# yynps737/zero-latency-yolo

Hardware: AMD Instinct MI355X
Metric: frames_per_sec (higher is better)
Workload: dtype bf16; 1 GPU; YOLOv8-nano 416x416 batch=64 throughput path (BASELINE configs[2]), bf16; engines_per_gpu=3, weights=seeded synthetic (no real weights offline), graph=True, parallelism=single GPU

## Files before the change

### zero-latency-yolo_amd/csrc/engine.cpp

```cpp
#include "zly_internal.h"
#include "weights.h"

#include <algorithm>
#include <atomic>
#include <chrono>
#include <condition_variable>
#include <deque>
#include <map>
#include <mutex>
#include <string>
#include <thread>
#include <type_traits>
#include <vector>
#include <string.h>
#include <stdio.h>
#include <stdlib.h>

namespace zly {

static thread_local std::string g_last_error;

static int fail(int code, const std::string& msg) { g_last_error = msg; return code; }

#define HIP_TRY(expr, code)                                                                        \
// ... 65 lines not shown
};

struct Plan {
    int nc = 0, N = 0;
    std::vector<Buffer> bufs;
    std::vector<Op> ops;
    std::vector<PairGroup> pairs;
    std::vector<C2fGroup> c2fs;
    DetectTail tail;
    int in_buf = -1;
    std::map<std::string, std::pair<int, int>> tap_index;
    std::map<std::string, std::pair<int, int>> tap_final;
    bool stem_fused = false;
    bool stem1 = false;
    size_t stem_w = 0, stem_b = 0, m1_w = 0, m1_b = 0, stem_w0p = 0;
    int stem_out = -1, m1_out = -1;
    int sppf_cv1 = -1, sppf_pool = -1, sppf_cv2 = -1;
    int det_stem[3] = {-1, -1, -1}, det_a[3] = {-1, -1, -1}, det_b[3] = {-1, -1, -1};
    bool det_merge_ok = false;
    int join_at = -1;
    std::vector<uint8_t> blob;
};

enum LaunchKind { LK_NONE, LK_PREPROCESS, LK_STEM, LK_STEM1, LK_CONV, LK_CONV_WSK, LK_MULTI, LK_C2F, LK_PAIR, LK_WS_PAIR, LK_SPPF_FUSED, LK_SPPF_POOL, LK_HEAD, LK_NMS };
struct Launch {
    int kind = LK_NONE;
    int covered_by = -1;
    bool hbm = true;
    ConvPlan conv{};
    WskPlan wsk{};
    C2fPlan c2f{};
    PairPlan pair{};
    WsPairPlan ws_pair{};
    int multi_ct = 0;
    int only_level = -1;
    int box_mode[3] = {0, 0, 0};
    bool pool16 = false;
    bool lb = false;
};

struct Ingest;

}

using namespace zly;

struct zly_engine : Plan {
    zly_config cfg;
    std::string weights_path;
    int dev = 0;
    int dtype = ZLY_DTYPE_BF16;
    size_t esz = 2;
    ModelFile model;

    void* d_weights = nullptr;
    float* d_head = nullptr;
    Cand* d_cand = nullptr;
    Cand* d_scratch = nullptr;
    int* d_count = nullptr;
// ... 60 lines not shown

namespace zly {

static size_t slab_bytes_of(const zly_engine* e) { return sizeof(zly_slab_header) + (size_t)e->cfg.max_dets * sizeof(zly_det); }

template <typename F> static void with_stats(zly_engine* e, F&& f) { std::lock_guard<std::mutex> lk(e->stats_mu); f(e->stats); }

static void read_switches(Switches* sw)
{
    auto on = [](const char* name) { return getenv(name) != nullptr; };
    auto num = [](const char* name, auto* out) { if (const char* v = getenv(name)) *out = (std::remove_pointer_t<decltype(out)>)atoll(v); };
    *sw = Switches();
    if (const char* cp = getenv("ZLY_CU_PART")) {
        int pi = 0, pn = 1;
        if (sscanf(cp, "%d/%d", &pi, &pn) == 2 && pn >= 1 && pn <= 8 && pi >= 0 && pi < pn) { sw->cu_part_i = pi; sw->cu_part_n = pn; sw->num_cus = 256 / pn; }
    }
    sw->no_lanes = on("ZLY_NO_LANES") || on("ZLY_CU_PART");
    sw->no_c2f = on("ZLY_NO_C2F");
    sw->no_det_merge = on("ZLY_NO_DET_MERGE");
    sw->no_tail_split = on("ZLY_NO_TAIL_SPLIT");
    num("ZLY_TAIL_BOX", &sw->tail_box);
    if (const char* v = getenv("ZLY_TAIL_BOX_MIN_CONF")) sw->tail_box_min_conf = (float)atof(v);
    sw->sppf_fused = on("ZLY_SPPF_FUSED");
    sw->pool_six_pass = on("ZLY_SPPF_POOL_LDS");
    sw->no_wsk = on("ZLY_NO_WSK");
    sw->nms_general = on("ZLY_NMS_GENERAL");
    sw->no_cout_pad = on("ZLY_NO_COUT_PAD");
    sw->no_cin_pad = on("ZLY_NO_CIN_PAD");
    sw->no_stem1 = on("ZLY_NO_STEM1");
    num("ZLY_STEM1_NW", &sw->stem1_nw);
    num("ZLY_STEM1_VAR", &sw->stem1_var);
    num("ZLY_STEM1_GRID", &sw->stem1_grid);
    num("ZLY_STEM1_TW", &sw->stem1_tw);
    num("ZLY_STEM1_TH", &sw->stem1_th);
    sw->stem1_keep_tiles = on("ZLY_STEM1_TW") || on("ZLY_STEM1_TH") || on("ZLY_STEM1_BIG_TILES");
    num("ZLY_PAIR_MIN_TILES", &sw->pair_min_tiles);
    num("ZLY_PAIR_WIDTHS", &sw->pair_widths);
    auto num_nonempty = [&](const char* name, int* out) { const char* v = getenv(name); if (v && *v) *out = atoi(v); };
    num_nonempty("ZLY_STAGE_SLOTS", &sw->stage_slots);
    num_nonempty("ZLY_STAGE_MB", &sw->stage_mb);
    num_nonempty("ZLY_INFLIGHT", &sw->inflight);
    { int d = 0; num_nonempty("ZLY_D2H_STREAM", &d); sw->d2h_stream = d != 0; }
    num("ZLY_PROFILE_INNER", &sw->profile_inner);
    if (sw->profile_inner < 1) sw->profile_inner = 1;
#ifdef ZLY_DIAG
    if (const char* v = getenv("ZLY_ABLATE_SKIP")) sw->ablate = std::string(",") + v + ",";
// ... 327 lines not shown
    p->stem1 = p->stem_fused && ch[0] == 16 && ch[1] == 32 && !(cfg.flags & ZLY_FLAG_NO_FUSION) && !sw.no_stem1 && ok;
    if (p->stem1) {
        const ConvRec* r = m.find("model.1");
        int cout_pad = 0, nk = 0;
        pb.pack(r, ch[0], 16, true, 4, nullptr, &p->m1_w, &p->m1_b, &nk, &cout_pad);
        if (nk != 9 || cout_pad != 32 || r->k != 3 || r->stride != 2) p->stem1 = false;
    }
    if (p->stem1) {
        int cout_pad = 0, nk0 = 0;
        pb.pack(m.find("model.0"), 4, pb.kstep, false, 0, stem1_tap_slot(), &p->stem_w0p, nullptr, &nk0, &cout_pad);
        if (nk0 != 2 || cout_pad != 16) p->stem1 = false;
    }
    ok = ok && pb.c2f("model.2", View{a1, 0, ch[1]}, View{a2, 0, ch[1]}, nb[0], true, H4, W4);
    ok = ok && pb.conv({"model.3"}, View{a2, 0, ch[1]}, View{a3, 0, ch[2]}) >= 0;
    ok = ok && pb.c2f("model.4", View{a3, 0, ch[2]}, View{cat14, ch[3], ch[2]}, nb[1], true, H8, W8);
    ok = ok && pb.conv({"model.5"}, View{cat14, ch[3], ch[2]}, View{a5, 0, ch[3]}) >= 0;
    ok = ok && pb.c2f("model.6", View{a5, 0, ch[3]}, View{cat11, ch[4], ch[3]}, nb[2], true, H16, W16);
    ok = ok && pb.conv({"model.7"}, View{cat11, ch[4], ch[3]}, View{a7, 0, ch[4]}) >= 0;
    ok = ok && pb.c2f("model.8", View{a7, 0, ch[4]}, View{a8, 0, ch[4]}, nb[3], true, H32, W32);
    ok = ok && (p->sppf_cv1 = pb.conv({"model.9.cv1"}, View{a8, 0, ch[4]}, View{spp, 0, ch[4] / 2})) >= 0;
    if (ok) {
        Op pool; pool.kind = OP_SPPF; pool.name = "model.9.pool"; pool.in = View{spp, 0, ch[4] / 2};
        pool.bytes = (double)H32 * W32 * (ch[4] / 2) * 4 * esz;
        p->sppf_pool = pb.add_op(pool);
    }
    ok = ok && (p->sppf_cv2 = pb.conv({"model.9.cv2"}, View{spp, 0, 2 * ch[4]}, View{cat20, ch[3], ch[4]})) >= 0;
    ok = ok && pb.c2f("model.12", View{cat20, ch[3], ch[4]}, View{cat17, ch[2], ch[3]}, nb[4], false, H16, W16, View{cat11, ch[4], ch[3]});
    ok = ok && pb.c2f("model.15", View{cat17, ch[2], ch[3]}, View{a15, 0, ch[2]}, nb[5], false, H8, W8, View{cat14, ch[3], ch[2]});
    ok = ok && pb.detect_level(0, View{a15, 0, ch[2]}, c2, c3, tail_total);
    ok = ok && pb.conv({"model.16"}, View{a15, 0, ch[2]}, View{cat17, 0, ch[2]}) >= 0;
    ok = ok && pb.c2f("model.18", View{cat17, 0, ch[2] + ch[3]}, View{a18, 0, ch[3]}, nb[6], false, H16, W16);
    ok = ok && pb.detect_level(1, View{a18, 0, ch[3]}, c2, c3, tail_total);
    ok = ok && pb.conv({"model.19"}, View{a18, 0, ch[3]}, View{cat20, 0, ch[3]}) >= 0;
    ok = ok && pb.c2f("model.21", View{cat20, 0, ch[3] + ch[4]}, View{a21, 0, ch[4]}, nb[7], false, H32, W32);
    ok = ok && pb.detect_level(2, View{a21, 0, ch[4]}, c2, c3, tail_total);
    if (!ok) return refuse(pb.err);
    Op nm; nm.kind = OP_NMS; nm.name = "nms"; pb.add_op(nm);
    return ZLY_OK;
}

static int upload_plan(zly_engine* e, std::string* err)
{
    const int W = e->cfg.model_w, H = e->cfg.model_h;
    const int B = e->cfg.max_batch;
    for (Buffer& b : e->bufs) {
        if (b.elems_per_frame() * (size_t)B >= (1ull << 31)) { *err = "activation buffer " + b.name + " exceeds 2^31 elements: lower max_batch"; return ZLY_ERR_INVALID_ARGUMENT; }
        const size_t bytes = b.elems_per_frame() * (b.f32 ? 4 : e->esz) * (size_t)B;
// ... 77 lines not shown
    ConvArgs k = make_conv_args(e, op, n);
    k.Cin = 80; k.K = 9 * 80; k.nk = 23; k.cout_pad = 80;
    k.wgt = (const char*)e->d_weights + op.wsk_w;
    return k;
}

static SppfArgs make_sppf_args(const zly_engine* e, int n)
{
    const Op& op = e->ops[(size_t)e->sppf_cv1];
    const Op& o2 = e->ops[(size_t)e->sppf_cv2];
    const Buffer& ib = e->bufs[(size_t)op.in.buf];
    const Buffer& cb = e->bufs[(size_t)op.out.buf];
    const Buffer& ob2 = e->bufs[(size_t)o2.out.buf];
    const char* wb = (const char*)e->d_weights;
    SppfArgs sa{};
    sa.x = ib.ptr; sa.x_cs = ib.C; sa.x_co = op.in.co; sa.Cin = op.in.C;
    sa.w1 = wb + op.w_off; sa.b1 = (const float*)(wb + op.b_off);
    sa.w2 = wb + o2.w_off; sa.b2 = (const float*)(wb + o2.b_off);
    sa.out = ob2.ptr; sa.out_cs = ob2.C; sa.out_co = o2.out.co; sa.Cout = o2.cout;
    sa.cat = cb.ptr; sa.cat_cs = cb.C;
    sa.H = cb.H; sa.W = cb.W; sa.n = n; sa.c = op.cout; sa.split = sppf_split(o2.cout, n, e->sw);
    sa.dump = (e->cfg.flags & ZLY_FLAG_DUMP_LOGITS) ? 1 : 0;
    return sa;
}

static PairArgs make_pair_args(const zly_engine* e, const PairGroup& g, const PairPlan& pl, int n)
{
    const Op& A = e->ops[(size_t)g.first];
    const Buffer& ib = e->bufs[(size_t)A.in.buf];
    const Buffer& ob = e->bufs[(size_t)g.out.buf];
    const char* wb = (const char*)e->d_weights;
    PairArgs pa;
    pa.in = ib.ptr; pa.in_cs = ib.C; pa.in_co = A.in.co;
    pa.out = ob.ptr; pa.out_cs = ob.C; pa.out_co = g.out.co;
    pa.wA = wb + g.wA; pa.bA = (const float*)(wb + g.bA);
    pa.wB = wb + g.wB; pa.bB = (const float*)(wb + g.bB);
    pa.H = ib.H; pa.W = ib.W; pa.n = n;
    pa.TH = pl.th; pa.TW = pl.tw; pa.tiles_x = pl.tiles_x; pa.tiles_y = pl.tiles_y; pa.total_tiles = pl.total_tiles;
    pa.res = g.res;
    return pa;
}

static C2fArgs make_c2f_args(const zly_engine* e, const C2fGroup& g, const C2fPlan& pl, int n)
{
    const PairGroup& pg = e->pairs[(size_t)g.pair];
    const Buffer& cb = e->bufs[(size_t)g.cat];
// ... 36 lines not shown
        const PairGroup& g = e->pairs[(size_t)A.pair];
        if (g.first != a || !(e->sw.pair_widths & g.c)) return false;
        const Buffer& b = e->bufs[(size_t)A.in.buf];
        return pair_plan(g.c, n, b.H, b.W, e->sw, pl) && pl->total_tiles >= e->sw.pair_min_tiles;
    };
    auto ws_pair_of = [&](int a, WsPairPlan* pl) {
        const Op& A = e->ops[(size_t)a];
        if (A.pair < 0 || !fusion) return false;
        const PairGroup& g = e->pairs[(size_t)A.pair];
        if (g.first != a || g.c != 64 || (e->sw.pair_widths & 64)) return false;
        const ConvArgs ca = make_conv_args(e, A, n), cb = make_conv_args(e, e->ops[(size_t)g.second], n);
        ConvPlan pa{}, pb{};
        conv_plan(e->dtype, 3, ca, e->sw, &pa);
        conv_plan(e->dtype, 3, cb, e->sw, &pb);
        return conv_ws_pair_plan(ca, cb, pa, pb, e->sw, pl);
    };
    bool sppf = fusion && e->sw.sppf_fused && e->sppf_cv1 >= 0;
    if (sppf) {
        const Op& a = e->ops[(size_t)e->sppf_cv1];
        const Op& b = e->ops[(size_t)e->sppf_cv2];
        sppf = a.act && b.act && a.res.buf < 0 && b.res.buf < 0 && a.in2.buf < 0 && b.in.C == 4 * a.cout && a.cout_pad == a.cout && b.cout_pad == b.cout &&
               sppf_fused_ok(make_sppf_args(e, n));
    }
    const bool merge = bf16 && e->det_merge_ok && n <= 4 && !lanes_active(e, n) && !e->sw.no_det_merge;
    auto merged_at = [&](int i) {
        for (int l = 0; l < 3; ++l) {
            if (i == e->det_stem[l]) return e->det_stem[2];
            if (i == e->det_a[l] || i == e->det_b[l]) return e->det_a[2];
        }
        return -1;
    };
    const bool tail_split = lanes_active(e, n) && !e->sw.no_tail_split;
    const int tail = e->tail.op[2];
    auto tail_box_mode = [&](int l) {
        const int ai = e->det_a[l];
        if (!bf16 || !fusion || e->sw.tail_box == 0 || ai < 0 || merge) return 0;
        if (e->sw.tail_box != 2 && (dump || !(e->cfg.flags & ZLY_FLAG_NO_HEAD_TENSOR) || e->cfg.conf_thr < e->sw.tail_box_min_conf)) return 0;
        const Op& op = e->ops[(size_t)ai];
        const Buffer& sb = e->bufs[(size_t)e->tail.stem[l]];
        if (op.ks != 3 || op.stride != 1 || !op.act || op.in.C != 64 || op.cout != 64 || op.cout_pad != 64 || op.nk != 18 || op.res.buf >= 0 || op.in.co != 0 || op.pair >= 0 || op.c2f >= 0) return 0;
        if ((size_t)n * sb.H * sb.W * sb.C * 2 >= ((size_t)1 << 31)) return 0;
        ConvPlan cp{};
        conv_plan(e->dtype, op.ks, make_conv_args(e, op, n), e->sw, &cp);
        if (cp.ksplit > 1) return 0;
        if (cp.kind == CONV_WS && !cp.rowt) return 1;
        if (cp.kind == CONV_LDS) return 2;
        return 0;
    };
    const int box_mode[3] = {tail_box_mode(0), tail_box_mode(1), tail_box_mode(2)};
    auto box_level = [&](int i) { for (int l = 0; l < 3; ++l) if (i == e->det_a[l] && box_mode[l]) return l; return -1; };

    const bool lb = (e->cfg.flags & ZLY_FLAG_LETTERBOX) != 0;
    std::vector<Launch> t((size_t)nops);
    for (int i = 0; i < nops; ++i) {
        const Op& op = e->ops[(size_t)i];
        Launch& L = t[(size_t)i];
        L.covered_by = i;
        L.lb = lb && (op.kind == OP_PREPROCESS || op.kind == OP_HEAD || (i == 1 && e->stem_fused));
        auto covered = [&](int by) { L.kind = LK_NONE; L.covered_by = by; };
        switch (op.kind) {
        case OP_PREPROCESS:
            if (e->stem_fused) covered(1);
            else L.kind = LK_PREPROCESS;
            break;
        case OP_SPPF: {
            const Buffer& b = e->bufs[(size_t)op.in.buf];
            if (sppf) covered(e->sppf_cv1);
            else { L.kind = LK_SPPF_POOL; L.pool16 = sppf_pool16_ok(e->dtype, b.C, op.in.C, n, b.H, b.W, e->sw.pool_six_pass ? 1 : 0); }
            break;
        }
        case OP_HEAD:
            if (tail_split || op.level == 2) { L.kind = LK_HEAD; L.only_level = tail_split ? op.level : -1; for (int l = 0; l < 3; ++l) L.box_mode[l] = box_mode[l]; }
            else covered(tail);
            break;
        case OP_NMS:
            L.kind = LK_NMS;
            break;
        case OP_CONV: {
            conv_plan(e->dtype, op.ks, make_conv_args(e, op, n), e->sw, &L.conv);
            C2fPlan cp{};
            PairPlan pp{};
            WsPairPlan wp{};
            if (i == 1 && e->stem_fused) {
                L.kind = e->stem1 ? LK_STEM1 : LK_STEM;
                L.hbm = !e->stem1 || dump;
            } else if (i == 2 && e->stem1) {
                covered(1);
            } else if (op.c2f >= 0 && c2f_of(e->c2fs[(size_t)op.c2f], &cp)) {
                const C2fGroup& g = e->c2fs[(size_t)op.c2f];
                if (g.leader == i) { L.kind = LK_C2F; L.c2f = cp; }
                else covered(g.leader);
                L.hbm = g.vis_of(i) == 0 || (g.vis_of(i) == 1 && dump);
            } else if (sppf && i == e->sppf_cv1) {
                L.kind = LK_SPPF_FUSED;
                L.hbm = dump;
            } else if (sppf && i == e->sppf_cv2) {
                covered(e->sppf_cv1);
            } else if (box_level(i) >= 0) {
                covered(tail_split ? e->tail.op[box_level(i)] : tail);
                L.hbm = dump;
            } else if (merge && merged_at(i) >= 0) {
                if (merged_at(i) == i) { L.kind = LK_MULTI; L.multi_ct = i == e->det_stem[2] ? 3 : 2; }
                else covered(merged_at(i));
            } else if (pair_of(i, &pp)) {
                L.kind = LK_PAIR; L.pair = pp;
                L.hbm = false;
            } else if (op.pair >= 0 && e->pairs[(size_t)op.pair].second == i && pair_of(e->pairs[(size_t)op.pair].first, &pp)) {
                covered(e->pairs[(size_t)op.pair].first);
            } else if (ws_pair_of(i, &wp)) {
                L.kind = LK_WS_PAIR; L.ws_pair = wp;
                L.hbm = dump;
            } else if (op.pair >= 0 && e->pairs[(size_t)op.pair].second == i && ws_pair_of(e->pairs[(size_t)op.pair].first, &wp)) {
                covered(e->pairs[(size_t)op.pair].first);
            } else if (op.wsk_w && !e->sw.no_wsk && bf16 && conv_wsk_ok(make_wsk_args(e, op, n), e->sw, &L.wsk)) {
                L.kind = LK_CONV_WSK;
            } else {
                L.kind = LK_CONV;
            }
            break;
        }
// ... 59 lines not shown
        return launch_conv_wsk(make_wsk_args(e, op, n), L.wsk, s);
    case LK_MULTI: {
        ConvArgsMulti m{};
        for (int l = 0; l < 3; ++l) {
            if (L.multi_ct == 3) m.a[m.n++] = make_conv_args(e, e->ops[(size_t)e->det_stem[l]], n);
            else { m.a[m.n++] = make_conv_args(e, e->ops[(size_t)e->det_a[l]], n); m.a[m.n++] = make_conv_args(e, e->ops[(size_t)e->det_b[l]], n); }
        }
        return launch_conv_multi(m, L.multi_ct, s);
    }
    case LK_C2F: {
        const C2fGroup& g = e->c2fs[(size_t)op.c2f];
        return launch_c2f(g.c, g.mode, make_c2f_args(e, g, L.c2f, n), L.c2f, s);
    }
    case LK_PAIR: {
        const PairGroup& g = e->pairs[(size_t)op.pair];
        return launch_pair(g.c, make_pair_args(e, g, L.pair, n), L.pair, s);
    }
    case LK_WS_PAIR: {
        const PairGroup& g = e->pairs[(size_t)op.pair];
        return launch_conv_ws_pair(make_conv_args(e, op, n), make_conv_args(e, e->ops[(size_t)g.second], n), L.ws_pair, (e->cfg.flags & ZLY_FLAG_DUMP_LOGITS) != 0, s);
    }
    case LK_SPPF_FUSED:
        return launch_sppf_fused(make_sppf_args(e, n), s);
    case LK_SPPF_POOL: {
        const Buffer& b = e->bufs[(size_t)op.in.buf];
        return launch_sppf_pool(e->dtype, b.ptr, b.C, op.in.C, n, b.H, b.W, s, e->sw.pool_six_pass ? 1 : 0);
    }
    case LK_HEAD: {
        HeadArgs h = e->tail.args;
        h.only_level = L.only_level;
        for (int l = 0; l < 3; ++l) {
            if (!L.box_mode[l]) continue;
            const Buffer& sb = e->bufs[(size_t)e->tail.stem[l]];
            h.lv[l].box_mode = L.box_mode[l]; h.lv[l].box_in = sb.ptr; h.lv[l].box_cs = sb.C;
        }
        if (L.lb) { h.lb_tw = e->cfg.model_w; h.lb_th = e->cfg.model_h; }
        h.head = (e->cfg.flags & ZLY_FLAG_NO_HEAD_TENSOR) ? nullptr : e->d_head; h.desc = e->d_desc; h.conf_thr = e->cfg.conf_thr; h.cand = e->cur_cand; h.cand_count = e->cur_count;
        return launch_head_fused(e->dtype, h, n, s);
    }
    case LK_NMS:
        return launch_nms(e->cur_cand, e->cur_count, e->N, n, e->cfg.iou_thr, e->nc, e->d_scratch,
                          d_slabs_out ? d_slabs_out : e->d_slabs, e->cfg.max_dets, tag0, s, e->sw.nms_general ? 1 : 0);
    }
    return hipErrorInvalidValue;
}

// ... 1418 lines not shown
{
    if (!e || !out || i < 0 || i >= (int32_t)e->ops.size()) return fail(ZLY_ERR_INVALID_ARGUMENT, "bad argument");
    const Op& op = e->ops[(size_t)i];
    memset(out, 0, sizeof *out);
    snprintf(out->name, sizeof out->name, "%s", op.name.c_str());
    out->kind = op.kind;
    out->flops_per_frame = op.flops;
    out->bytes_per_frame = op.bytes;
    return ZLY_OK;
}

int32_t zly_op_kernel_name(zly_engine* e, int32_t i, int32_t n, char* out, size_t cap)
{
    if (!e || !out || cap < 8 || i < 0 || i >= (int32_t)e->ops.size() || n < 1 || n > e->cfg.max_batch) return fail(ZLY_ERR_INVALID_ARGUMENT, "bad argument");
    std::lock_guard<std::mutex> lk(e->mu);
    const std::vector<Launch>& t = resolve_launches(e, n);
    const Launch& L = t[(size_t)i];
    const Op& op = e->ops[(size_t)i];
    std::string k;
    switch (L.kind) {
    case LK_NONE:
        switch (t[(size_t)L.covered_by].kind) {
        case LK_STEM: case LK_STEM1: k = op.kind == OP_PREPROCESS ? "(fused into stem_fused_kernel)" : "(fused into the previous launch)"; break;
        case LK_PAIR: case LK_WS_PAIR: k = "(fused into the previous launch)"; break;
        case LK_C2F: k = "(fused into the C2f kernel at " + e->ops[(size_t)L.covered_by].name + ")"; break;
        case LK_SPPF_FUSED: k = "(fused into the SPPF kernel at model.9.cv1)"; break;
        case LK_MULTI: k = "(in a merged Detect launch)"; break;
        case LK_HEAD: k = op.kind == OP_CONV ? "(computed in the Detect tail at surviving anchors)" : "(covered by the last tail launch)"; break;
        }
        break;
    case LK_PREPROCESS: k = L.lb ? "preprocess_kernel<LB> (letterbox)" : "preprocess_kernel"; break;
    case LK_STEM: k = L.lb ? "stem_fused_kernel<LB> (letterbox)" : "stem_fused_kernel"; break;
    case LK_STEM1: k = L.lb ? "stem_model1_kernel<LB> (letterbox preprocess+model.0+model.1)" : "stem_model1_kernel (preprocess+model.0+model.1)"; break;
    case LK_SPPF_POOL: k = L.pool16 ? "sppf_pool16_kernel<DPP row windows, one barrier>" : "sppf_pool_kernel"; break;
    case LK_SPPF_FUSED: k = "sppf_fused_kernel<cv1+3 pools+cv2,SPLIT=" + std::to_string(sppf_split(e->ops[(size_t)e->sppf_cv2].cout, n, e->sw)) + ">"; break;
    case LK_MULTI: k = L.multi_ct == 3 ? "conv_igemm_multi_kernel<CT=3> (the 3 Detect stems)" : "conv_igemm_multi_kernel<CT=2> (the 6 Detect branch convs)"; break;
    case LK_C2F: {
        const C2fGroup& g = e->c2fs[(size_t)op.c2f];
        k = "c2f_kernel<C=" + std::to_string(g.c) + (g.c == 32 ? ",NW=" + std::to_string(L.c2f.nw) : std::string()) +
            (g.mode == 3 ? ",cv1+bottleneck+cv2>" : g.mode == 1 ? ",cv1+bottleneck>" : ",bottleneck+cv2>");
        break;
    }
    case LK_PAIR: k = "bottleneck_pair_kernel<" + std::to_string(e->pairs[(size_t)op.pair].c) + ">"; break;
    case LK_WS_PAIR: k = std::string("conv3x3_ws_pair_kernel<") + (e->pairs[(size_t)op.pair].res ? "RES," : "") + "64->64->64," + std::to_string(L.ws_pair.g.TH) + "x" + std::to_string(L.ws_pair.g.TW) + " tiles>"; break;
    case LK_CONV_WSK: k = "conv3x3_wsk_kernel<K=720 packed across taps,5 channel tiles>"; break;
    case LK_CONV: {
        const int cin = op.in.C + (op.in2.buf >= 0 ? op.in2.C : 0);
        const ConvPlan& c = L.conv;
        switch (c.kind) {
        case CONV_WS1: k = std::string("conv1x1_ws_kernel<") + (op.in2.buf >= 0 ? "dual-source," : "") + "NK=" + std::to_string(cin / 32) + "," + std::to_string(c.ct) + " channel tiles," + std::to_string(c.pt * 16) + " px>"; break;
        case CONV_WS: k = std::string("conv3x3_ws_kernel<") + (op.stride == 2 ? "S=2," : "") + (c.rowt ? "ROWT," : "") + (c.tpw1 ? "TPW=1," : "TPW=2,") + std::to_string(c.ct) + " channel tiles>"; break;
        case CONV_LDS: k = "conv3x3_lds_kernel<S=" + std::to_string(op.stride) + ",CT=" + std::to_string(c.ct) + ",PT=" + std::to_string(c.pt) + (c.wres ? ",wres>" : ">"); break;
        case CONV_STREAM: k = "conv1x1_stream_kernel<CT=" + std::to_string(c.ct) + ",PT=" + std::to_string(c.pt) + ",NK=" + std::to_string((cin + 31) / 32) + ">"; break;
        default: k = std::string("conv_igemm_kernel<") + (op.ks == 1 ? (op.in2.buf >= 0 ? "1x1 dual-source" : "1x1") : (c.fastk ? "3x3" : "3x3 generic-K")) +
                 ",CT=" + std::to_string(c.ct) + ",PT=" + std::to_string(c.pt) + ",KSPLIT=" + std::to_string(c.ksplit) + ">";
        }
        break;
    }
// ... 143 lines not shown
```

### zero-latency-yolo_amd/csrc/kernels_misc.hip

```cpp
#include "zly_internal.h"
#include "yuv_device.h"
#include "letterbox_device.h"

namespace zly {

typedef __attribute__((ext_vector_type(8))) __bf16 bf16x8;
typedef __attribute__((ext_vector_type(4))) float f32x4;

template <typename T, bool YUV, bool LB = false, bool VIEW = false, bool PK = false>
__global__ __launch_bounds__(256) void preprocess_kernel(const uint8_t* __restrict__ src, const FrameDesc* __restrict__ desc,
                                                         T* __restrict__ out8, float* __restrict__ out_nchw, int tw, int th)
{
    const int f = blockIdx.y;
    const int idx = blockIdx.x * 256 + threadIdx.x;
    if (idx >= tw * th) return;
    const int y = idx / tw, x = idx - y * tw;
    const FrameDesc d = desc[f];
    const float scale_w = (float)d.w / (float)tw;
    const float scale_h = (float)d.h / (float)th;
    int sy = (int)((float)y * scale_h); if (sy > d.h - 1) sy = d.h - 1;
    int sx = (int)((float)x * scale_w); if (sx > d.w - 1) sx = d.w - 1;
    const Planes<VIEW> pl = frame_planes<VIEW, PK>(src, src + (YUV ? desc_off(d.src_off) : d.src_off), desc, (int)gridDim.y, f, d, YUV ? desc_fmt(d.src_off) : ZLY_PIX_BGR);
    float b, g, r;
    if constexpr (LB) {
        const int fmt = YUV ? desc_fmt(d.src_off) : ZLY_PIX_BGR;
// ... 158 lines not shown
            for (int d = 1; d <= 2; ++d) {
                if (x - d >= 0) m = px_max(m, row[x - d]);
                if (x + d < W) m = px_max(m, row[x + d]);
            }
            R[px] = m;
        }
        __syncthreads();
        for (int px = threadIdx.x; px < hw; px += 256) {
            const int y = px / W, x = px - y * W;
            Px8 m = R[px];
#pragma unroll
            for (int d = 1; d <= 2; ++d) {
                if (y - d >= 0) m = px_max(m, R[(y - d) * W + x]);
                if (y + d < H) m = px_max(m, R[(y + d) * W + x]);
            }
            B[px] = m;
            store_px8(base + (size_t)px * cs + stage * c, m);
        }
        __syncthreads();
        Px8* t = A; A = B; B = t;
    }
}

typedef __attribute__((ext_vector_type(4))) unsigned int pu32x4;
typedef __attribute__((ext_vector_type(8))) short ps16x8;
__device__ __forceinline__ pu32x4 pool_sortable(pu32x4 v)
{
    pu32x4 r;
#pragma unroll
    for (int i = 0; i < 4; ++i) { const unsigned sg = v[i] & 0x80008000u; r[i] = v[i] ^ (sg - (sg >> 15)); }
    return r;
}
__device__ __forceinline__ pu32x4 pool_max(pu32x4 a, pu32x4 b)
{
    return __builtin_bit_cast(pu32x4, __builtin_elementwise_max(__builtin_bit_cast(ps16x8, a), __builtin_bit_cast(ps16x8, b)));
}
template <int CTRL> __device__ __forceinline__ pu32x4 pool_row_shift(pu32x4 v)
{
    pu32x4 r;
#pragma unroll
    for (int i = 0; i < 4; ++i) r[i] = (unsigned)__builtin_amdgcn_update_dpp((int)0x80008000u, (int)v[i], CTRL, 0xf, 0xf, false);
    return r;
}
__device__ __forceinline__ pu32x4 pool_row5(pu32x4 v)
{
    pu32x4 m = pool_max(v, pool_row_shift<0x111>(v));
    m = pool_max(m, pool_row_shift<0x112>(v));
    m = pool_max(m, pool_row_shift<0x101>(v));
    return pool_max(m, pool_row_shift<0x102>(v));
}
__global__ __launch_bounds__(256) void sppf_pool16_kernel(unsigned short* __restrict__ buf, int cs, int c, int H, int W)
{
    __shared__ __attribute__((aligned(16))) pu32x4 rows[3][16][16];
    const int x = threadIdx.x & 15, y = threadIdx.x >> 4;
    const int f = blockIdx.y, c0 = blockIdx.x * 8;
    const bool in = y < H && x < W;
    unsigned short* px = buf + ((size_t)f * H * W + (size_t)(in ? y * W + x : 0)) * cs + c0;
    const pu32x4 pad = {0x80008000u, 0x80008000u, 0x80008000u, 0x80008000u};
    pu32x4 v = pad;
    if (in) v = pool_sortable(*reinterpret_cast<const pu32x4*>(px));
    const pu32x4 r2 = pool_row5(v), r4 = pool_row5(r2), r6 = pool_row5(r4);
    rows[0][y][x] = r2; rows[1][y][x] = r4; rows[2][y][x] = r6;
    __syncthreads();
    if (!in) return;
    const int ymax = H - 1;
#pragma unroll
    for (int k = 0; k < 3; ++k) {
        const int rad = 2 * k + 2;
        pu32x4 m = rows[k][y][x];
#pragma unroll
        for (int d = 1; d <= rad; ++d) {
            m = pool_max(m, rows[k][max(y - d, 0)][x]);
            m = pool_max(m, rows[k][min(y + d, ymax)][x]);
// ... 57 lines not shown
```

### zero-latency-yolo_amd/csrc/kernels_sppf.hip

```cpp
#include "zly_internal.h"
#include "conv_device.h"

namespace zly {

typedef __attribute__((ext_vector_type(8))) short s16x8;

static constexpr int SPPF_C = 128;
static constexpr int SPPF_KC = SPPF_C / 32;
static constexpr int SPPF_NW = 16;
static constexpr int SPPF_TP = SPPF_C * 2 + 32;
static constexpr int SPPF_MAXPX = 176;

#ifdef ZLY_SPPF_DIAG
__device__ unsigned long long* g_sppf_diag = nullptr;
#define SPPFSTAMP(k) do { __builtin_amdgcn_sched_barrier(0); unsigned long long t_; asm volatile("s_memtime %0\n\ts_waitcnt lgkmcnt(0)" : "=s"(t_) :: "memory"); dsum[k] += t_ - dT0; dT0 = t_; __builtin_amdgcn_sched_barrier(0); } while (0)
#else
#define SPPFSTAMP(k) do { } while (0)
#endif

__device__ __forceinline__ u32x4 sortable(u32x4 v)
{
    u32x4 r;
#pragma unroll
    for (int i = 0; i < 4; ++i) { const unsigned sg = v[i] & 0x80008000u; r[i] = v[i] ^ (sg - (sg >> 15)); }
// ... 189 lines not shown
        if (j >= NCT || q >= HW) continue;
        f32x4 lo = acc2[jj][0] + b2lo, hi = acc2[jj][1] + b2hi;
#pragma unroll
        for (int r = 0; r < 4; ++r) { lo[r] = silu<bf16_t>(lo[r]); hi[r] = silu<bf16_t>(hi[r]); }
        *reinterpret_cast<bf16x8*>(out + ((size_t)(f * HW + q) * a.out_cs + a.out_co + ch)) = to_bf16x8(lo, hi);
    }
#ifdef ZLY_SPPF_DIAG
    if (lane == 0 && g_sppf_diag) {
        unsigned long long* o = g_sppf_diag + (((size_t)blockIdx.y * gridDim.x + blockIdx.x) * SPPF_NW + wave) * 16;
        for (int i = 0; i < 8; ++i) o[i] = dsum[i];
        o[8] = __builtin_amdgcn_s_memtime() - dstart;
    }
#endif
}

static size_t sppf_lds_bytes(int cin, int hw)
{
    (void)hw;
    const size_t phase1 = (size_t)SPPF_MAXPX * ((size_t)cin * 2 + 32) + (size_t)(SPPF_C / 16) * (cin / 32) * 1024;
    const size_t phase2 = (size_t)3 * SPPF_MAXPX * SPPF_TP;
    return phase1 > phase2 ? phase1 : phase2;
}

typedef void (*sppf_fn)(const SppfArgs);
static sppf_fn pick_sppf(int nk1, int np2)
{
    if (nk1 == 8) return np2 == 2 ? sppf_fused_kernel<8, 2> : np2 == 4 ? sppf_fused_kernel<8, 4> : nullptr;
    return nullptr;
}

int sppf_split(int cout, int n, const Switches& sw) { return (cout / 4) % 64 == 0 && (long)n * 4 <= (long)sw.num_cus ? 4 : 2; }

bool sppf_fused_ok(const SppfArgs& a)
{
    if (a.c != SPPF_C || a.Cin != 256 || a.Cout % 128 != 0 || a.Cout > 256 || a.H * a.W > SPPF_MAXPX || a.H < 3 || a.W < 3) return false;
    if (sppf_lds_bytes(a.Cin, a.H * a.W) > 160 * 1024) return false;
    if (a.x_cs % 8 || a.x_co % 8 || a.out_cs % 8 || a.out_co % 8 || a.cat_cs % 8 || a.n < 1 || (a.split != 2 && a.split != 4)) return false;
    if ((size_t)a.n * a.H * a.W * (size_t)std::max(a.x_cs, std::max(a.out_cs, a.cat_cs)) * 2 >= ((size_t)1 << 31)) return false;
    return pick_sppf(a.Cin / 32, a.Cout / a.split / 32) != nullptr;
}

hipError_t sppf_init()
{
    for (int np2 = 2; np2 <= 4; np2 += 2) {
        hipError_t r = hipFuncSetAttribute((const void*)pick_sppf(8, np2), hipFuncAttributeMaxDynamicSharedMemorySize, 160 * 1024);
        if (r != hipSuccess) return r;
    }
    return hipSuccess;
}

hipError_t launch_sppf_fused(const SppfArgs& a, hipStream_t s)
{
    if (!sppf_fused_ok(a)) return hipErrorInvalidValue;
    hipLaunchKernelGGL(pick_sppf(a.Cin / 32, a.Cout / a.split / 32), dim3(a.split, a.n), dim3(SPPF_NW * 64), sppf_lds_bytes(a.Cin, a.H * a.W), s, a);
    return hipGetLastError();
}

}
```

### zero-latency-yolo_amd/csrc/zly_internal.h

```cpp
#pragma once
#include <hip/hip_runtime.h>
#include <stdint.h>
#include <stddef.h>
#include <string>
#include "zly.h"

namespace zly {

typedef __bf16 bf16_t;

struct FrameDesc {
    unsigned long long src_off;
    int w, h;
};
#define ZLY_DESC_FMT_SHIFT 56
__host__ __device__ __forceinline__ unsigned long long desc_pack(unsigned long long off, int fmt) { return off | ((unsigned long long)fmt << ZLY_DESC_FMT_SHIFT); }
__host__ __device__ __forceinline__ unsigned long long desc_off(unsigned long long v) { return v & ((1ull << ZLY_DESC_FMT_SHIFT) - 1); }
__host__ __device__ __forceinline__ int desc_fmt(unsigned long long v) { return (int)(v >> ZLY_DESC_FMT_SHIFT); }

#define ZLY_FRONT_BGR    0
#define ZLY_FRONT_YUV    1
#define ZLY_FRONT_PACKED 2
__host__ __device__ __forceinline__ int front_level(int fmt)
{
// ... 22 lines not shown
    int Cin;
    int in2_cs, in2_co, split_c;
    int K;
    void* out;        int out_cs, out_co;
    int Cout;
    const void* res;  int res_cs, res_co;
    int act;
    int out_f32;
};

struct ConvArgsMulti { ConvArgs a[6]; int n; };
hipError_t launch_conv_multi(const ConvArgsMulti& m, int ct, hipStream_t s);

struct Switches {
    int  num_cus = 256;
    int  cu_part_i = 0, cu_part_n = 1;
    bool no_lanes = false;
    bool no_c2f = false;
    bool no_det_merge = false;
    bool no_tail_split = false;
    int  tail_box = 1;
    float tail_box_min_conf = 0.05f;
    bool sppf_fused = false;
    bool pool_six_pass = false;
    bool no_wsk = false;
    bool nms_general = false;
    bool no_cout_pad = false;
    bool no_cin_pad = false;
    bool no_stem1 = false;
    int  stem1_nw = 0;
    int  stem1_var = 1;
    int  stem1_grid = 0;
    int  stem1_tw = 0, stem1_th = 0;
    bool stem1_keep_tiles = false;
    int  pair_min_tiles = 32;
    int  pair_widths = 48;
    int  stage_slots = 6;
    int  stage_mb = 0;
    int  inflight = 2;
    bool d2h_stream = false;
    int  profile_inner = 1;
    std::string ablate;
    bool no_stream = false;
    bool stream_ct2 = false;
    int  stream_max_nk = 1 << 30;
    long stream_min_groups = 4096;
// ... 127 lines not shown
    int small_tiles;
    float inv_pw, inv_rw, inv_tw, inv_qb;
    const void* wgt0p;
};
void       stem1_plan(int H1, int W1, const Switches& sw, int* th, int* tw);
hipError_t stem1_init();
hipError_t launch_stem_model1(const Stem1Args& a, int n, hipStream_t s, int yuv = 0, bool lb = false, bool view = false);
const int* stem1_tap_slot();

struct SppfArgs {
    const void* x; int x_cs, x_co, Cin;
    const void* w1; const float* b1;
    const void* w2; const float* b2;
    void* out; int out_cs, out_co, Cout;
    void* cat; int cat_cs;
    int H, W, n, c;
    int split;
    int dump;
};
bool       sppf_fused_ok(const SppfArgs& a);
int        sppf_split(int cout, int n, const Switches& sw);
hipError_t sppf_init();
hipError_t launch_sppf_fused(const SppfArgs& a, hipStream_t s);

struct HeadLevel {
    const void* box_in; const void* cls_in;
    int box_cs, cls_cs, box_cin, cls_cin;
    const void* wb; const void* wc;
    const float* bb; const float* bc;
    int nkb, nkc;
    int H, W, hw, stride_px, anchor_off, block0;
    float* logits; int logits_cs;
    int box_mode;
    const void* w1; const float* b1;
    void* box2;
};
#define HEAD_KMAX 8
#define HEAD_WAVES 8
#define HEAD_GROUP (HEAD_WAVES * 16)
struct HeadArgs {
    HeadLevel lv[3];
    int nc, N_total, total_blocks;
    int only_level;
    float* head;
    const FrameDesc* desc; float conf_thr;
    float skip_logit;
// ... 16 lines not shown
```

Baseline: 116,100 frames/s.

## Fuse SPPF cv1 conv with the three max-pools into one kernel

After: 116,900 frames/s (median of 6 runs). No clear change (+0.7%).

```diff
diff --git a/zero-latency-yolo_amd/csrc/engine.cpp b/zero-latency-yolo_amd/csrc/engine.cpp
--- a/zero-latency-yolo_amd/csrc/engine.cpp
+++ b/zero-latency-yolo_amd/csrc/engine.cpp
@@ -111,7 +111,7 @@
     std::vector<uint8_t> blob;
 };
 
-enum LaunchKind { LK_NONE, LK_PREPROCESS, LK_STEM, LK_STEM1, LK_CONV, LK_CONV_WSK, LK_MULTI, LK_C2F, LK_PAIR, LK_WS_PAIR, LK_SPPF_FUSED, LK_SPPF_POOL, LK_HEAD, LK_NMS };
+enum LaunchKind { LK_NONE, LK_PREPROCESS, LK_STEM, LK_STEM1, LK_CONV, LK_CONV_WSK, LK_MULTI, LK_C2F, LK_PAIR, LK_WS_PAIR, LK_SPPF_FUSED, LK_SPPF_HEAD, LK_SPPF_POOL, LK_HEAD, LK_NMS };
 struct Launch {
     int kind = LK_NONE;
     int covered_by = -1;
@@ -124,6 +124,7 @@
     int multi_ct = 0;
     int only_level = -1;
     int box_mode[3] = {0, 0, 0};
+    SppfHeadPlan sppf_head{};
     bool pool16 = false;
     bool lb = false;
 };
@@ -230,6 +231,7 @@
     num("ZLY_TAIL_BOX", &sw->tail_box);
     if (const char* v = getenv("ZLY_TAIL_BOX_MIN_CONF")) sw->tail_box_min_conf = (float)atof(v);
     sw->sppf_fused = on("ZLY_SPPF_FUSED");
+    num("ZLY_SPPF_HEAD", &sw->sppf_head);
     sw->pool_six_pass = on("ZLY_SPPF_POOL_LDS");
     sw->no_wsk = on("ZLY_NO_WSK");
     sw->nms_general = on("ZLY_NMS_GENERAL");
@@ -603,7 +605,10 @@
     if (ok) {
         Op pool; pool.kind = OP_SPPF; pool.name = "model.9.pool"; pool.in = View{spp, 0, ch[4] / 2};
         pool.bytes = (double)H32 * W32 * (ch[4] / 2) * 4 * esz;
+        pool.out = View{spp, ch[4] / 2, 3 * (ch[4] / 2)};
+        for (int k = 0; k < 3; ++k) { pool.taps.push_back("model.9.pool." + std::to_string(k + 1)); pool.tap_co.push_back(k * (ch[4] / 2)); pool.tap_c.push_back(ch[4] / 2); }
         p->sppf_pool = pb.add_op(pool);
+        for (int k = 0; k < 3; ++k) p->tap_index[pool.taps[(size_t)k]] = std::make_pair(p->sppf_pool, k);
     }
     ok = ok && (p->sppf_cv2 = pb.conv({"model.9.cv2"}, View{spp, 0, 2 * ch[4]}, View{cat20, ch[3], ch[4]})) >= 0;
     ok = ok && pb.c2f("model.12", View{cat20, ch[3], ch[4]}, View{cat17, ch[2], ch[3]}, nb[4], false, H16, W16, View{cat11, ch[4], ch[3]});
@@ -727,6 +732,20 @@
     sa.H = cb.H; sa.W = cb.W; sa.n = n; sa.c = op.cout; sa.split = sppf_split(o2.cout, n, e->sw);
     sa.dump = (e->cfg.flags & ZLY_FLAG_DUMP_LOGITS) ? 1 : 0;
     return sa;
+}
+
+static SppfHeadArgs make_sppf_head_args(const zly_engine* e, int n)
+{
+    const Op& op = e->ops[(size_t)e->sppf_cv1];
+    const Buffer& ib = e->bufs[(size_t)op.in.buf];
+    const Buffer& cb = e->bufs[(size_t)op.out.buf];
+    const char* wb = (const char*)e->d_weights;
+    SppfHeadArgs ha{};
+    ha.x = ib.ptr; ha.x_cs = ib.C; ha.x_co = op.in.co;
+    ha.w1 = wb + op.w_off; ha.b1 = (const float*)(wb + op.b_off);
+    ha.cat = cb.ptr; ha.cat_cs = cb.C; ha.cat_co = op.out.co;
+    ha.H = cb.H; ha.W = cb.W; ha.n = n; ha.c = op.cout;
+    return ha;
 }
 
 static PairArgs make_pair_args(const zly_engine* e, const PairGroup& g, const PairPlan& pl, int n)
@@ -809,6 +828,18 @@
         sppf = a.act && b.act && a.res.buf < 0 && b.res.buf < 0 && a.in2.buf < 0 && b.in.C == 4 * a.cout && a.cout_pad == a.cout && b.cout_pad == b.cout &&
                sppf_fused_ok(make_sppf_args(e, n));
     }
+    SppfHeadPlan head_plan{};
+    bool sppf_head = fusion && !sppf && e->sppf_cv1 >= 0 && e->sppf_pool == e->sppf_cv1 + 1 && (e->sw.sppf_head == 2 || (e->sw.sppf_head == 1 && n > 16));
+    if (sppf_head) {
+        const Op& a = e->ops[(size_t)e->sppf_cv1];
+        const Op& pl = e->ops[(size_t)e->sppf_pool];
+        ConvPlan cp{};
+        conv_plan(e->dtype, a.ks, make_conv_args(e, a, n), e->sw, &cp);
+        const int order = (cp.kind == CONV_WS1 || (cp.kind == CONV_DIRECT && cp.ksplit == 1)) ? 1 : (cp.kind == CONV_DIRECT && cp.ksplit == 4 && a.nk % 4 == 0) ? 4 : 0;
+        sppf_head = order && a.ks == 1 && a.stride == 1 && a.act && !a.out_f32 && a.res.buf < 0 && a.in2.buf < 0 && a.cout_pad == a.cout && a.nk * 32 == a.in.C &&
+                    pl.in.buf == a.out.buf && pl.in.co == a.out.co && pl.in.C == a.cout &&
+                    sppf_head_ok(e->dtype, make_sppf_head_args(e, n), a.in.C, 32, order, &head_plan);
+    }
     const bool merge = bf16 && e->det_merge_ok && n <= 4 && !lanes_active(e, n) && !e->sw.no_det_merge;
     auto merged_at = [&](int i) {
         for (int l = 0; l < 3; ++l) {
@@ -852,7 +883,7 @@
             break;
         case OP_SPPF: {
             const Buffer& b = e->bufs[(size_t)op.in.buf];
-            if (sppf) covered(e->sppf_cv1);
+            if (sppf || sppf_head) { covered(e->sppf_cv1); L.hbm = sppf_head || dump; }
             else { L.kind = LK_SPPF_POOL; L.pool16 = sppf_pool16_ok(e->dtype, b.C, op.in.C, n, b.H, b.W, e->sw.pool_six_pass ? 1 : 0); }
             break;
         }
@@ -883,6 +914,8 @@
                 L.hbm = dump;
             } else if (sppf && i == e->sppf_cv2) {
                 covered(e->sppf_cv1);
+            } else if (sppf_head && i == e->sppf_cv1) {
+                L.kind = LK_SPPF_HEAD; L.sppf_head = head_plan;
             } else if (box_level(i) >= 0) {
                 covered(tail_split ? e->tail.op[box_level(i)] : tail);
                 L.hbm = dump;
@@ -988,6 +1021,8 @@
     }
     case LK_SPPF_FUSED:
         return launch_sppf_fused(make_sppf_args(e, n), s);
+    case LK_SPPF_HEAD:
+        return launch_sppf_head(make_sppf_head_args(e, n), L.sppf_head, s);
     case LK_SPPF_POOL: {
         const Buffer& b = e->bufs[(size_t)op.in.buf];
         return launch_sppf_pool(e->dtype, b.ptr, b.C, op.in.C, n, b.H, b.W, s, e->sw.pool_six_pass ? 1 : 0);
@@ -2452,7 +2487,7 @@
     case LK_NONE:
         switch (t[(size_t)L.covered_by].kind) {
         case LK_STEM: case LK_STEM1: k = op.kind == OP_PREPROCESS ? "(fused into stem_fused_kernel)" : "(fused into the previous launch)"; break;
-        case LK_PAIR: case LK_WS_PAIR: k = "(fused into the previous launch)"; break;
+        case LK_PAIR: case LK_WS_PAIR: case LK_SPPF_HEAD: k = "(fused into the previous launch)"; break;
         case LK_C2F: k = "(fused into the C2f kernel at " + e->ops[(size_t)L.covered_by].name + ")"; break;
         case LK_SPPF_FUSED: k = "(fused into the SPPF kernel at model.9.cv1)"; break;
         case LK_MULTI: k = "(in a merged Detect launch)"; break;
@@ -2464,6 +2499,7 @@
     case LK_STEM1: k = L.lb ? "stem_model1_kernel<LB> (letterbox preprocess+model.0+model.1)" : "stem_model1_kernel (preprocess+model.0+model.1)"; break;
     case LK_SPPF_POOL: k = L.pool16 ? "sppf_pool16_kernel<DPP row windows, one barrier>" : "sppf_pool_kernel"; break;
     case LK_SPPF_FUSED: k = "sppf_fused_kernel<cv1+3 pools+cv2,SPLIT=" + std::to_string(sppf_split(e->ops[(size_t)e->sppf_cv2].cout, n, e->sw)) + ">"; break;
+    case LK_SPPF_HEAD: k = "sppf_cv1_pool_kernel<cv1+3 pools,NK1=" + std::to_string(L.sppf_head.nk1) + ",SL=" + std::to_string(L.sppf_head.sl) + (L.sppf_head.ksplit == 4 ? ",split-K order>" : ",ascending k>"); break;
     case LK_MULTI: k = L.multi_ct == 3 ? "conv_igemm_multi_kernel<CT=3> (the 3 Detect stems)" : "conv_igemm_multi_kernel<CT=2> (the 6 Detect branch convs)"; break;
     case LK_C2F: {
         const C2fGroup& g = e->c2fs[(size_t)op.c2f];
diff --git a/zero-latency-yolo_amd/csrc/kernels_misc.hip b/zero-latency-yolo_amd/csrc/kernels_misc.hip
--- a/zero-latency-yolo_amd/csrc/kernels_misc.hip
+++ b/zero-latency-yolo_amd/csrc/kernels_misc.hip
@@ -1,6 +1,7 @@
 #include "zly_internal.h"
 #include "yuv_device.h"
 #include "letterbox_device.h"
+#include "pool_device.h"
 
 namespace zly {
 
@@ -205,33 +206,6 @@
     }
 }
 
-typedef __attribute__((ext_vector_type(4))) unsigned int pu32x4;
-typedef __attribute__((ext_vector_type(8))) short ps16x8;
-__device__ __forceinline__ pu32x4 pool_sortable(pu32x4 v)
-{
-    pu32x4 r;
-#pragma unroll
-    for (int i = 0; i < 4; ++i) { const unsigned sg = v[i] & 0x80008000u; r[i] = v[i] ^ (sg - (sg >> 15)); }
-    return r;
-}
-__device__ __forceinline__ pu32x4 pool_max(pu32x4 a, pu32x4 b)
-{
-    return __builtin_bit_cast(pu32x4, __builtin_elementwise_max(__builtin_bit_cast(ps16x8, a), __builtin_bit_cast(ps16x8, b)));
-}
-template <int CTRL> __device__ __forceinline__ pu32x4 pool_row_shift(pu32x4 v)
-{
-    pu32x4 r;
-#pragma unroll
-    for (int i = 0; i < 4; ++i) r[i] = (unsigned)__builtin_amdgcn_update_dpp((int)0x80008000u, (int)v[i], CTRL, 0xf, 0xf, false);
-    return r;
-}
-__device__ __forceinline__ pu32x4 pool_row5(pu32x4 v)
-{
-    pu32x4 m = pool_max(v, pool_row_shift<0x111>(v));
-    m = pool_max(m, pool_row_shift<0x112>(v));
-    m = pool_max(m, pool_row_shift<0x101>(v));
-    return pool_max(m, pool_row_shift<0x102>(v));
-}
 __global__ __launch_bounds__(256) void sppf_pool16_kernel(unsigned short* __restrict__ buf, int cs, int c, int H, int W)
 {
     __shared__ __attribute__((aligned(16))) pu32x4 rows[3][16][16];
diff --git a/zero-latency-yolo_amd/csrc/kernels_sppf.hip b/zero-latency-yolo_amd/csrc/kernels_sppf.hip
--- a/zero-latency-yolo_amd/csrc/kernels_sppf.hip
+++ b/zero-latency-yolo_amd/csrc/kernels_sppf.hip
@@ -1,5 +1,6 @@
 #include "zly_internal.h"
 #include "conv_device.h"
+#include "pool_device.h"
 
 namespace zly {
 
@@ -235,6 +236,190 @@
     return phase1 > phase2 ? phase1 : phase2;
 }
 
+template <int NK1, int SL, int KS>
+__global__ __launch_bounds__(256, 2) void sppf_cv1_pool_kernel(const SppfHeadArgs a)
+{
+    extern __shared__ __attribute__((aligned(16))) unsigned char smem[];
+    constexpr int NT = SL / 16;
+    constexpr int NG = SL / 32;
+    constexpr int PP = SL * 2;
+    constexpr int PER = NK1 / KS;
+    constexpr bool AHEAD = NK1 <= 8;
+    const int tid = threadIdx.x, lane = tid & 63;
+    const int wave = __builtin_amdgcn_readfirstlane(tid >> 6);
+    const int p = lane & 15, kq = lane >> 4;
+    const int f = blockIdx.y, c0 = blockIdx.x * SL;
+    const int HW = a.H * a.W, NCT = (HW + 15) >> 4;
+    const int plane = a.H * 16 * PP;
+#ifdef ZLY_SPPF_DIAG
+    unsigned long long dsum[8] = {0, 0, 0, 0, 0, 0, 0, 0}, dT0 = __builtin_amdgcn_s_memtime();
+    const unsigned long long dstart = dT0;
+#endif
+
+    bf16x8 w[NT][NK1];
+    {
+        const bf16_t* __restrict__ wb = static_cast<const bf16_t*>(a.w1) + lane * 8;
+        const int tile0 = blockIdx.x * NT;
+#pragma unroll
+        for (int t = 0; t < NT; ++t)
+#pragma unroll
+            for (int s = 0; s < NK1; ++s) w[t][s] = *reinterpret_cast<const bf16x8*>(wb + ((size_t)(tile0 + t) * NK1 + s) * 512);
+    }
+    f32x4 biasr[NT];
+#pragma unroll
+    for (int t = 0; t < NT; ++t) biasr[t] = *reinterpret_cast<const f32x4*>(a.b1 + c0 + (t >> 1) * 32 + kq * 8 + (t & 1) * 4);
+    const bf16_t* __restrict__ xin = static_cast<const bf16_t*>(a.x) + a.x_co + (size_t)f * HW * a.x_cs + kq * 8;
+    bf16_t* __restrict__ cat = static_cast<bf16_t*>(a.cat) + a.cat_co + (size_t)f * HW * a.cat_cs + c0;
+    auto load_x = [&](int j, bf16x8 (&xf)[NK1]) {
+        const int q = min(j * 16 + p, HW - 1);
+        const bf16_t* xp = xin + (size_t)q * a.x_cs;
+#pragma unroll
+        for (int s = 0; s < NK1; ++s) xf[s] = *reinterpret_cast<const bf16x8*>(xp + s * 32);
+    };
+    auto tile = [&](int j, const bf16x8 (&xf)[NK1]) {
+        f32x4 acc[NT];
+        if constexpr (KS == 1) {
+#pragma unroll
+            for (int t = 0; t < NT; ++t) acc[t] = f32x4{0.f, 0.f, 0.f, 0.f};
+#pragma unroll
+            for (int s = 0; s < NK1; ++s)
+#pragma unroll
+                for (int t = 0; t < NT; ++t) acc[t] = mma_step(w[t][s], xf[s], acc[t]);
+        } else {
+            f32x4 part[KS][NT];
+#pragma unroll
+            for (int k = 0; k < KS; ++k)
+#pragma unroll
+                for (int t = 0; t < NT; ++t) part[k][t] = f32x4{0.f, 0.f, 0.f, 0.f};
+#pragma unroll
+            for (int s = 0; s < NK1; ++s)
+#pragma unroll
+                for (int t = 0; t < NT; ++t) part[s / PER][t] = mma_step(w[t][s], xf[s], part[s / PER][t]);
+#pragma unroll
+            for (int t = 0; t < NT; ++t) {
+                acc[t] = part[0][t];
+#pragma unroll
+                for (int k = 1; k < KS; ++k) acc[t] += part[k][t];
+            }
+        }
+        const int q = j * 16 + p;
+        const int yy = (int)(((float)q + 0.5f) * a.inv_w), xx = q - yy * a.W;
+#pragma unroll
+        for (int g = 0; g < NG; ++g) {
+            f32x4 lo = acc[2 * g] + biasr[2 * g], hi = acc[2 * g + 1] + biasr[2 * g + 1];
+#pragma unroll
+            for (int r = 0; r < 4; ++r) { lo[r] = silu<bf16_t>(lo[r]); hi[r] = silu<bf16_t>(hi[r]); }
+            const bf16x8 yv = to_bf16x8(lo, hi);
+            if (q < HW) {
+                *reinterpret_cast<bf16x8*>(cat + (size_t)q * a.cat_cs + g * 32 + kq * 8) = yv;
+                *reinterpret_cast<pu32x4*>(smem + (yy * 16 + xx) * PP + g * 64 + kq * 16) = pool_sortable(__builtin_bit_cast(pu32x4, yv));
+            }
+        }
+    };
+    if constexpr (AHEAD) {
+        bf16x8 xa[NK1], xb[NK1];
+        if (wave < NCT) load_x(wave, xa);
+#pragma unroll
+        for (int jj = 0; jj < 4; ++jj) {
+            const int j = wave + jj * 4;
+            if (j < NCT) {
+                if (j + 4 < NCT) load_x(j + 4, (jj & 1) ? xa : xb);
+                tile(j, (jj & 1) ? xb : xa);
+            }
+        }
+    } else {
+        for (int j = wave; j < NCT; j += 4) {
+            bf16x8 xf[NK1];
+            load_x(j, xf);
+            tile(j, xf);
+        }
+    }
+    SPPFSTAMP(0);
+    __syncthreads();
+    SPPFSTAMP(1);
+
+    const pu32x4 pad = {0x80008000u, 0x80008000u, 0x80008000u, 0x80008000u};
+    const bool in = p < a.W;
+    for (int y = wave; y < a.H; y += 4) {
+#pragma unroll
+        for (int g = 0; g < NG; ++g) {
+            unsigned char* cell = smem + (y * 16 + p) * PP + g * 64 + kq * 16;
+            pu32x4 v = pad;
+            if (in) v = *reinterpret_cast<const pu32x4*>(cell);
+            const pu32x4 r2 = pool_row5(v), r4 = pool_row5(r2), r6 = pool_row5(r4);
+            *reinterpret_cast<pu32x4*>(cell) = r2;
+            *reinterpret_cast<pu32x4*>(cell + plane) = r4;
+            *reinterpret_cast<pu32x4*>(cell + 2 * plane) = r6;
+        }
+    }
+    SPPFSTAMP(2);
+    __syncthreads();
+    SPPFSTAMP(3);
+    const int ymax = a.H - 1;
+    for (int y = wave; y < a.H; y += 4) {
+        if (!in) continue;
+        bf16_t* px = cat + (size_t)(y * a.W + p) * a.cat_cs + kq * 8;
+#pragma unroll
+        for (int g = 0; g < NG; ++g) {
+#pragma unroll
+            for (int k = 0; k < 3; ++k) {
+                const int rad = 2 * k + 2;
+                const unsigned char* col = smem + k * plane + p * PP + g * 64 + kq * 16;
+                pu32x4 m = *reinterpret_cast<const pu32x4*>(col + y * 16 * PP);
+#pragma unroll
+                for (int d = 1; d <= rad; ++d) {
+                    m = pool_max(m, *reinterpret_cast<const pu32x4*>(col + max(y - d, 0) * 16 * PP));
+                    m = pool_max(m, *reinterpret_cast<const pu32x4*>(col + min(y + d, ymax) * 16 * PP));
+                }
+                *reinterpret_cast<pu32x4*>(px + (size_t)(k + 1) * a.c + g * 32) = pool_sortable(m);
+            }
+        }
+    }
+    SPPFSTAMP(4);
+#ifdef ZLY_SPPF_DIAG
+    if (lane == 0 && g_sppf_diag) {
+        unsigned long long* o = g_sppf_diag + (((size_t)blockIdx.y * gridDim.x + blockIdx.x) * 4 + wave) * 16;
+        for (int i = 0; i < 8; ++i) o[i] = dsum[i];
+        o[8] = __builtin_amdgcn_s_memtime() - dstart;
+    }
+#endif
+}
+
+typedef void (*sppf_head_fn)(const SppfHeadArgs);
+static sppf_head_fn pick_sppf_head(int nk1, int sl, int ks)
+{
+#define ZLY_SPPF_HEAD_CASE(N_, S_) if (nk1 == N_ && sl == S_) return ks == 1 ? sppf_cv1_pool_kernel<N_, S_, 1> : ks == 4 ? sppf_cv1_pool_kernel<N_, S_, 4> : nullptr
+    ZLY_SPPF_HEAD_CASE(8, 32);
+#ifdef ZLY_SPPF_DIAG
+    if (nk1 == 8 && sl == 64 && ks == 1) return sppf_cv1_pool_kernel<8, 64, 1>;
+#endif
+    ZLY_SPPF_HEAD_CASE(16, 32);
+#undef ZLY_SPPF_HEAD_CASE
+    return nullptr;
+}
+static constexpr unsigned SPPF_HEAD_LDS_MAX = 3 * 16 * 16 * 64 * 2;
+
+bool sppf_head_ok(int dtype, const SppfHeadArgs& a, int cin, int sl, int ksplit, SppfHeadPlan* plan)
+{
+    if (dtype != ZLY_DTYPE_BF16 || a.H < 1 || a.W < 1 || a.H > 16 || a.W > 16 || a.n < 1 || a.n > 65535 || sl < 32 || a.c < sl || a.c % sl || cin % 32) return false;
+    if (a.x_cs % 8 || a.x_co % 8 || a.cat_cs % 8 || a.cat_co % 8 || a.x_co + cin > a.x_cs || a.cat_co + 4 * a.c > a.cat_cs) return false;
+    const sppf_head_fn fn = pick_sppf_head(cin / 32, sl, ksplit);
+    if (!fn) return false;
+    plan->nk1 = cin / 32; plan->sl = sl; plan->ksplit = ksplit;
+    plan->lds = (unsigned)(3 * a.H * 16 * sl * 2);
+    plan->fn = (const void*)fn;
+    return plan->lds <= SPPF_HEAD_LDS_MAX;
+}
+
+hipError_t launch_sppf_head(const SppfHeadArgs& a, const SppfHeadPlan& plan, hipStream_t s)
+{
+    if (!plan.fn || plan.lds > SPPF_HEAD_LDS_MAX) return hipErrorInvalidValue;
+    SppfHeadArgs b = a;
+    b.inv_w = 1.0f / (float)a.W;
+    hipLaunchKernelGGL(reinterpret_cast<sppf_head_fn>(const_cast<void*>(plan.fn)), dim3(a.c / plan.sl, a.n), dim3(256), plan.lds, s, b);
+    return hipGetLastError();
+}
+
 typedef void (*sppf_fn)(const SppfArgs);
 static sppf_fn pick_sppf(int nk1, int np2)
 {
@@ -259,6 +444,12 @@
         hipError_t r = hipFuncSetAttribute((const void*)pick_sppf(8, np2), hipFuncAttributeMaxDynamicSharedMemorySize, 160 * 1024);
         if (r != hipSuccess) return r;
     }
+#ifdef ZLY_SPPF_DIAG
+    {
+        hipError_t r = hipFuncSetAttribute((const void*)pick_sppf_head(8, 64, 1), hipFuncAttributeMaxDynamicSharedMemorySize, (int)SPPF_HEAD_LDS_MAX);
+        if (r != hipSuccess) return r;
+    }
+#endif
     return hipSuccess;
 }
 
diff --git a/zero-latency-yolo_amd/csrc/pool_device.h b/zero-latency-yolo_amd/csrc/pool_device.h
--- /dev/null
+++ b/zero-latency-yolo_amd/csrc/pool_device.h
@@ -0,0 +1,34 @@
+#pragma once
+#include "zly_internal.h"
+
+namespace zly {
+
+typedef __attribute__((ext_vector_type(4))) unsigned int pu32x4;
+typedef __attribute__((ext_vector_type(8))) short ps16x8;
+__device__ __forceinline__ pu32x4 pool_sortable(pu32x4 v)
+{
+    pu32x4 r;
+#pragma unroll
+    for (int i = 0; i < 4; ++i) { const unsigned sg = v[i] & 0x80008000u; r[i] = v[i] ^ (sg - (sg >> 15)); }
+    return r;
+}
+__device__ __forceinline__ pu32x4 pool_max(pu32x4 a, pu32x4 b)
+{
+    return __builtin_bit_cast(pu32x4, __builtin_elementwise_max(__builtin_bit_cast(ps16x8, a), __builtin_bit_cast(ps16x8, b)));
+}
+template <int CTRL> __device__ __forceinline__ pu32x4 pool_row_shift(pu32x4 v)
+{
+    pu32x4 r;
+#pragma unroll
+    for (int i = 0; i < 4; ++i) r[i] = (unsigned)__builtin_amdgcn_update_dpp((int)0x80008000u, (int)v[i], CTRL, 0xf, 0xf, false);
+    return r;
+}
+__device__ __forceinline__ pu32x4 pool_row5(pu32x4 v)
+{
+    pu32x4 m = pool_max(v, pool_row_shift<0x111>(v));
+    m = pool_max(m, pool_row_shift<0x112>(v));
+    m = pool_max(m, pool_row_shift<0x101>(v));
+    return pool_max(m, pool_row_shift<0x102>(v));
+}
+
+}
diff --git a/zero-latency-yolo_amd/csrc/zly_internal.h b/zero-latency-yolo_amd/csrc/zly_internal.h
--- a/zero-latency-yolo_amd/csrc/zly_internal.h
+++ b/zero-latency-yolo_amd/csrc/zly_internal.h
@@ -68,6 +68,7 @@
     int  tail_box = 1;
     float tail_box_min_conf = 0.05f;
     bool sppf_fused = false;
+    int  sppf_head = 1;
     bool pool_six_pass = false;
     bool no_wsk = false;
     bool nms_general = false;
@@ -241,6 +242,16 @@
 int        sppf_split(int cout, int n, const Switches& sw);
 hipError_t sppf_init();
 hipError_t launch_sppf_fused(const SppfArgs& a, hipStream_t s);
+struct SppfHeadArgs {
+    const void* x; int x_cs, x_co;
+    const void* w1; const float* b1;
+    void* cat; int cat_cs, cat_co;
+    int H, W, n, c;
+    float inv_w;
+};
+struct SppfHeadPlan { int nk1, sl, ksplit; unsigned lds; const void* fn; };
+bool       sppf_head_ok(int dtype, const SppfHeadArgs& a, int cin, int sl, int ksplit, SppfHeadPlan* plan);
+hipError_t launch_sppf_head(const SppfHeadArgs& a, const SppfHeadPlan& plan, hipStream_t s);
 
 struct HeadLevel {
     const void* box_in; const void* cls_in;
```
